# Xinran1205/LBM-Asynchronous

Measured on AMD Instinct MI355X. Metric: MLUPS, higher is better.
Workload: dtype f32

## Files before the change

lbm-asynchronous_amd/csrc/lbm_hip.hip:

```cpp
#include "../../include/lbm_hip.h"
#include "lbm_kernels.hip.h"

#include <hip/hip_runtime.h>
#include <hip/hip_ext.h>
#include <rccl/rccl.h>

#include <dlfcn.h>
#include <algorithm>

#include <atomic>
#include <condition_variable>
#include <cstdarg>
#include <cstdio>
#include <cstdlib>
#include <cstring>
#include <functional>
#include <mutex>
#include <thread>
#include <vector>

namespace {

constexpr int kMaxSlabs = 8;
constexpr int kPartSlots = lbm::kPartSlotsMax;
// ... 91 lines not shown
  LBM_RCCL_SYM(Recv, "ncclRecv");                    LBM_RCCL_SYM(AllReduce, "ncclAllReduce");
  LBM_RCCL_SYM(GetErrorString, "ncclGetErrorString");
#undef LBM_RCCL_SYM
  if (!ok) { r.handle = nullptr; return; }
  Dl_info di;
  if (dladdr(reinterpret_cast<void*>(r.GetVersion), &di) && di.dli_fname) {
    char real[512];
    const char* shown = realpath(di.dli_fname, real) ? real : di.dli_fname;
    strncpy(r.path, shown, sizeof(r.path) - 1);
  }
}

RcclApi* rccl() {
  std::call_once(g_rccl_once, rccl_bind);
  return g_rccl.handle ? &g_rccl : nullptr;
}

#define RCCL_OR_FAIL(ret)                                                       \
  RcclApi* rc_api_ = rccl();                                                    \
  if (!rc_api_) LBM_FAIL(ret, "RCCL is not available: %s", g_rccl_error)

constexpr int kMaxBandGroups = 3;

struct Slab {
  int device = 0;
  int row_first = 0;
  int rows = 0;
  int accel_row = lbm::kNoRow;
  int accel_row2 = lbm::kNoRow;
  float* lat_alloc[2] = {nullptr, nullptr};
  float* lat[2] = {nullptr, nullptr};
  unsigned char* mask_alloc = nullptr;
  unsigned char* mask = nullptr;
  float* partials = nullptr;
  double* tot_u = nullptr;
  double* scratch = nullptr;
  double* reduce_buf = nullptr;
  int* flushed_dev = nullptr;
  uint4* res_gran = nullptr;
  float* res_part = nullptr;
  int* res_status = nullptr;
  int* res_status_host = nullptr;
  float* frames = nullptr;
  lbm::probe_vec* probe_ring = nullptr;
  lbm::ProbeEntry* probe_table = nullptr;
  int probe_count = 0;
  hipGraphExec_t chunk_graph[2] = {nullptr, nullptr};
  hipStream_t compute = nullptr, comm = nullptr;
  hipEvent_t ev_boundary = nullptr, ev_halo = nullptr, ev_t0 = nullptr, ev_t1 = nullptr;
  hipEvent_t ev_interior[2] = {nullptr, nullptr};
  hipEvent_t ev_flush = nullptr;
  hipEvent_t ev_step = nullptr;
  hipEvent_t ev_fork = nullptr;
  hipEvent_t ev_x[2] = {nullptr, nullptr};
  hipStream_t group_extra[kMaxBandGroups - 1] = {nullptr, nullptr};
  hipEvent_t ev_gi[2][kMaxBandGroups] = {};
  hipEvent_t ev_gs[2] = {nullptr, nullptr};
  float* fresh_stage = nullptr;
  unsigned* fresh_arrived = nullptr;
  unsigned* fresh_id_src = nullptr;
  int* fresh_decision = nullptr;
  unsigned char* fresh_log = nullptr;
  hipEvent_t ev_fresh[2] = {nullptr, nullptr};
  ncclComm_t nccl = nullptr;
  lbm::SlotCounts slot_counts;
  int blocks_main = 0;
// ... 122 lines not shown
  Slab slab[kMaxSlabs];
  int cur = 0;
  int steps_done = 0;
  int capacity = 0;
  int fluid_cells = 0;
  int math_mode = LBM_MATH_EXACT;
  int halo = HALO_SELF;
  int halo_mode = LBM_HALO_SYNC;
  int rank = 0, world = 1;
  bool ranked = false;
  bool hosted = false;
  lbm_host_comm host_comm = {nullptr, nullptr, nullptr};
  float* host_send[2] = {nullptr, nullptr};
  float* host_recv[2] = {nullptr, nullptr};
  int row_first = 0, row_count = 0;
  int slot_fill = 0;
  long part_stride = 0;
  bool vec4 = false;
  int neigh = 0;
  int nts = 1;
  int snake = 0;
  int fuse2 = 0;
  int pass_steps = 2;
  int prefetch = 0;
  int xcd_chunk = 0;
  int use_stepk = 0;
  int packed = 0;
  int halo_lanes = 1;
  int lds_windows = 0;
  int band_rows = 8, n_strips = 0;
  int band_groups = 1;
  bool groups_forked = false;
  int lane_cells = 4;
  SlabTeam* team = nullptr;
  int use_graph = 0;
  GraphBuilder* builder = nullptr;
  int resident = 0;
  int resident_min_steps = 16;
  int resident_bands = 0;
  int resident_joint = 0;
  int resident_rows = 4;
  int resident_group = 1;
  int resident_one_xcd = 0;
  long long resident_timeout = 0;
  bool resident_used = false;
  int tile_steps = 0;
  int tile_shape = 0;
  lbm_batch* batch = nullptr;
  int frame_every = 0;
  int frame_slots = 0;
  int frame_ord0 = 0;
  long long frames_written = 0;
  long long frames_read = 0;
  std::vector<lbm_probe> probe_cells;
  int probe_every = 0;
  int probe_slots = 0;
  int probe_ord0 = 0;
  long long probes_written = 0;
  long long probes_read = 0;
  lbm::SteadyState* steady_state = nullptr;
  int* steady_stop_host = nullptr;
  hipEvent_t ev_steady[2] = {nullptr, nullptr};
};

struct lbm_batch {
  std::vector<lbm_ctx*> members;
// ... 156 lines not shown
  return q_kernel(c, stream, reinterpret_cast<const void*>(kernel), dim3(waves), dim3(64), args, done);
}

int launch_stepk(lbm_ctx* c, int s, hipStream_t stream, int k, int row_first, int row_end, int band_rows,
                 int band_pitch, int band_count, int part_offset, bool accel_after, hipEvent_t done = nullptr) {
  Slab& sl = c->slab[s];
  if (band_count <= 0) return LBM_SUCCESS;
  lbm::StepKArgs a;
  a.src = sl.lat[c->cur];
  a.dst = sl.lat[c->cur ^ 1];
  a.mask = sl.mask;
  a.plane_stride = c->plane_stride;
  a.row_pitch = c->row_pitch;
  a.pitch = c->pitch;
  a.nx = c->p.nx;
  a.rows = sl.rows;
  a.wrap = (c->halo == HALO_SELF) ? 1 : 0;
  a.band_rows = band_rows;
  a.row_first = row_first;
  a.band_pitch = band_pitch;
  a.row_end = row_end;
  a.n_strips = c->n_strips;
  a.n_bands = band_count;
  a.chunk = c->xcd_chunk;
  a.halo_lanes = c->halo_lanes;
  a.accel_row = sl.accel_row;
  a.accel_row2 = sl.accel_row2;
  a.accel_after = accel_after ? 1 : 0;
  a.omega = c->p.omega;
  a.a1 = c->p.density * c->p.accel / 9.f;
  a.a2 = c->p.density * c->p.accel / 36.f;
  a.partials = sl.partials + (long)c->slot_fill * c->part_stride + part_offset;
  a.slot_stride = c->part_stride;
  int waves = c->n_strips * band_count;
  if (a.chunk > 0) {
    const int chunks = band_count * ceil_div(c->n_strips, a.chunk);
    waves = 8 * ceil_div(chunks, 8) * a.chunk;
  }
  typedef void (*fn)(const lbm::StepKArgs);
#define LBM_K_ROW(M, N) {{lbm::stepk_stream<M, N, 4, 2, false>, lbm::stepk_stream<M, N, 4, 2, true>}, \
                         {lbm::stepk_stream<M, N, 4, 3, false>, lbm::stepk_stream<M, N, 4, 3, true>}, \
                         {lbm::stepk_stream<M, N, 4, 4, false>, lbm::stepk_stream<M, N, 4, 4, false>}}
  static const fn table[2][2][3][2] = {{LBM_K_ROW(0, false), LBM_K_ROW(0, true)}, {LBM_K_ROW(1, false), LBM_K_ROW(1, true)}};
#undef LBM_K_ROW
#define LBM_PK(N, KK, PF) {lbm::stepk_pk<N, KK, (PF && KK < 4), 0>, lbm::stepk_pk<N, KK, (PF && KK < 4), 1>, lbm::stepk_pk<N, KK, PF, (KK > 2 ? 2 : 1)>}
#define LBM_PK_ROW(N) {{LBM_PK(N, 2, false), LBM_PK(N, 2, true)}, {LBM_PK(N, 3, false), LBM_PK(N, 3, true)}, \
                       {LBM_PK(N, 4, false), LBM_PK(N, 4, true)}}
  static const fn table_pk[2][3][2][3] = {LBM_PK_ROW(false), LBM_PK_ROW(true)};
#undef LBM_PK_ROW
#undef LBM_PK
#define LBM_PK1(N, KK, PF) {lbm::stepk_pk<N, KK, (PF && KK < 4), 0, false, 1>, lbm::stepk_pk<N, KK, PF, 1, false, 1>}
#define LBM_PK1_ROW(N) {{LBM_PK1(N, 2, false), LBM_PK1(N, 2, true)}, {LBM_PK1(N, 3, false), LBM_PK1(N, 3, true)}, \
                        {LBM_PK1(N, 4, false), LBM_PK1(N, 4, true)}}
  static const fn table_pk1[2][3][2][2] = {LBM_PK1_ROW(false), LBM_PK1_ROW(true)};
#undef LBM_PK1_ROW
#undef LBM_PK1
  const int lds_windows = c->lds_windows < k ? c->lds_windows : k - 1;
  const bool packed = c->packed != 0;
  const fn kernel = (packed && c->lane_cells == 2) ? table_pk1[c->nts][k - 2][c->prefetch ? 1 : 0][lds_windows ? 1 : 0]
                    : packed ? table_pk[c->nts][k - 2][c->prefetch ? 1 : 0][lds_windows]
                           : table[c->math_mode == LBM_MATH_EXACT ? 0 : 1][c->nts][k - 2][c->prefetch ? 1 : 0];
  void* args[] = {&a};
  return q_kernel(c, stream, reinterpret_cast<const void*>(kernel), dim3(waves), dim3(64), args, done);
}

int launch_pass(lbm_ctx* c, int s, hipStream_t stream, int k, int row_first, int row_end, int band_rows,
                int band_pitch, int band_count, int part_offset, bool accel_after, hipEvent_t done = nullptr) {
  if ((c->lane_cells == 4 && (k > 2 || c->prefetch || c->xcd_chunk || c->use_stepk || c->packed)) ||
      (c->lane_cells == 2 && c->packed))
    return launch_stepk(c, s, stream, k, row_first, row_end, band_rows, band_pitch, band_count, part_offset, accel_after, done);
  return launch_step2(c, s, stream, row_first, row_end, band_rows, band_pitch, band_count, part_offset, accel_after, done);
}

int tile_count_for(const lbm_params* p, int shape) {
  return ceil_div(p->nx, kTileShapes[shape].tw) * ceil_div(p->ny, kTileShapes[shape].th);
}
int tile_count(const lbm_ctx* c) {
  const TileShape& t = kTileShapes[c->tile_shape];
  return ceil_div(c->p.nx, t.tw) * ceil_div(c->slab[0].rows, t.th);
}

int launch_tile(lbm_ctx* c, hipStream_t stream, int n_steps, bool accel_after) {
  Slab& sl = c->slab[0];
  lbm::TileArgs a;
  a.src = sl.lat[c->cur];
  a.dst = sl.lat[c->cur ^ 1];
  a.mask = sl.mask;
  a.plane_stride = c->plane_stride;
  a.row_pitch = c->row_pitch;
  a.pitch = c->pitch;
  a.nx = c->p.nx;
  a.ny = sl.rows;
  a.n_steps = n_steps;
// ... 966 lines not shown
          return LBM_SUCCESS;
        }) != LBM_SUCCESS)
      return LBM_FAILURE;
    for (int s = 0; s < c->n_slabs; s++)
      c->slab[s].slot_counts.n[c->slot_fill] = freshest ? c->slab[s].blocks_main + c->slab[s].blocks_boundary : blocks_for_rows(c, c->slab[s].rows);
    c->cur ^= 1;
    c->slot_fill += 1;
    if (!last && freshest && !force_never && fresh_exchange(c, c->cur, (m + 1) & 1, (unsigned)(c->steps_done + m + 1) + 1u) != LBM_SUCCESS)
      return LBM_FAILURE;
    if (!last && exchange_halos(c, depth, c->cur, c->cur ^ 1, slot) != LBM_SUCCESS) return LBM_FAILURE;
    if (c->slot_fill >= kPartSlots - 1 || last) {
      if (flush_partials(c, flushed_upto) != LBM_SUCCESS) return LBM_FAILURE;
      flushed_upto += c->slot_fill;
      c->slot_fill = 0;
    }
  }
  c->steps_done += n_steps;

  for (int s = 0; s < c->n_slabs; s++) {
    Slab& sl = c->slab[s];
    HIP_TRY(LBM_FAILURE, hipSetDevice(sl.device));
    for (int i = 0; i < 2; i++) HIP_TRY(LBM_FAILURE, hipStreamWaitEvent(sl.compute, sl.ev_x[i], 0));
  }
  return kernel_ms ? read_step_timing(c, n_steps, kernel_ms) : LBM_SUCCESS;
}

void free_slab(Slab& sl) {
  if (hipSetDevice(sl.device) != hipSuccess) return;
  for (int i = 0; i < 2; i++)
    if (sl.chunk_graph[i]) { (void)hipGraphExecDestroy(sl.chunk_graph[i]); sl.chunk_graph[i] = nullptr; }
  if (sl.nccl && g_rccl.CommDestroy) g_rccl.CommDestroy(sl.nccl);
  for (int i = 0; i < 2; i++) if (sl.lat_alloc[i]) (void)hipFree(sl.lat_alloc[i]);
  if (sl.mask_alloc) (void)hipFree(sl.mask_alloc);
  if (sl.partials) (void)hipFree(sl.partials);
  if (sl.tot_u) (void)hipFree(sl.tot_u);
  if (sl.scratch) (void)hipFree(sl.scratch);
  if (sl.reduce_buf) (void)hipFree(sl.reduce_buf);
  if (sl.flushed_dev) (void)hipFree(sl.flushed_dev);
  if (sl.fresh_stage) (void)hipFree(sl.fresh_stage);
  if (sl.fresh_arrived) (void)hipFree(sl.fresh_arrived);
  if (sl.fresh_id_src) (void)hipFree(sl.fresh_id_src);
  if (sl.fresh_decision) (void)hipFree(sl.fresh_decision);
  if (sl.fresh_log) (void)hipFree(sl.fresh_log);
  for (int i = 0; i < 2; i++) if (sl.ev_fresh[i]) (void)hipEventDestroy(sl.ev_fresh[i]);
  if (sl.res_gran) (void)hipFree(sl.res_gran);
  if (sl.res_part) (void)hipFree(sl.res_part);
  if (sl.res_status) (void)hipFree(sl.res_status);
  if (sl.res_status_host) (void)hipHostFree(sl.res_status_host);
  if (sl.frames) (void)hipFree(sl.frames);
  if (sl.probe_ring) (void)hipFree(sl.probe_ring);
  if (sl.probe_table) (void)hipFree(sl.probe_table);
  if (sl.ev_boundary) (void)hipEventDestroy(sl.ev_boundary);
  if (sl.ev_halo) (void)hipEventDestroy(sl.ev_halo);
  for (int i = 0; i < 2; i++) if (sl.ev_interior[i]) (void)hipEventDestroy(sl.ev_interior[i]);
  if (sl.ev_flush) (void)hipEventDestroy(sl.ev_flush);
  if (sl.ev_step) (void)hipEventDestroy(sl.ev_step);
  if (sl.ev_fork) (void)hipEventDestroy(sl.ev_fork);
  for (int i = 0; i < 2; i++) if (sl.ev_x[i]) (void)hipEventDestroy(sl.ev_x[i]);
  if (sl.ev_t0) (void)hipEventDestroy(sl.ev_t0);
  if (sl.ev_t1) (void)hipEventDestroy(sl.ev_t1);
  for (int i = 0; i < 2; i++) {
    if (sl.ev_gs[i]) (void)hipEventDestroy(sl.ev_gs[i]);
    for (int g = 0; g < kMaxBandGroups; g++) if (sl.ev_gi[i][g]) (void)hipEventDestroy(sl.ev_gi[i][g]);
  }
  for (int g = 0; g < kMaxBandGroups - 1; g++) if (sl.group_extra[g]) (void)hipStreamDestroy(sl.group_extra[g]);
  if (sl.compute) (void)hipStreamDestroy(sl.compute);
// ... 73 lines not shown
      HIP_TRY(LBM_FAILURE, hipMalloc(&tile_buf.p, tn));
      unsigned char* tile_dev = tile_buf.as<unsigned char>();
      HIP_TRY(LBM_FAILURE, hipMemcpyAsync(tile_dev, t8.data(), tn, hipMemcpyHostToDevice, sl.compute));
      hipLaunchKernelGGL(lbm::mask_from_tile, dim3(ceil_div((long)p.nx * mrows, 256)), dim3(256), 0, sl.compute, tile_dev,
                         obst.tile_nx, obst.tile_ny, sl.mask_alloc, p.nx, c->pitch, sl.row_first - kMaskHalo, mrows, p.ny);
      HIP_TRY(LBM_FAILURE, hipGetLastError());
      HIP_TRY(LBM_FAILURE, hipStreamSynchronize(sl.compute));
    } else {
      long chunk_rows = (32L << 20) / ((long)p.nx * sizeof(int));
      if (chunk_rows < 1) chunk_rows = 1;
      DeviceTemp stage_buf;
      HIP_TRY(LBM_FAILURE, hipMalloc(&stage_buf.p, (size_t)chunk_rows * p.nx * sizeof(int)));
      int* stage = stage_buf.as<int>();
      for (int r = 0; r < mrows;) {
        long src_row;
        int run = mrows - r;
        if (obst.kind == OBST_ROWS) {
          src_row = (long)(sl.row_first - c->row_first) + r;
        } else {
          const int g = ((sl.row_first - kMaskHalo + r) % p.ny + p.ny) % p.ny;
          src_row = g;
          if (run > p.ny - g) run = p.ny - g;
        }
        if (run > chunk_rows) run = (int)chunk_rows;
        HIP_TRY(LBM_FAILURE, hipMemcpyAsync(stage, obst.data + (size_t)src_row * p.nx, (size_t)run * p.nx * sizeof(int),
                                            hipMemcpyHostToDevice, sl.compute));
        hipLaunchKernelGGL(lbm::mask_from_int, dim3(ceil_div((long)p.nx * run, 256)), dim3(256), 0, sl.compute, stage,
                           sl.mask_alloc + (size_t)r * c->pitch, p.nx, c->pitch, run);
        HIP_TRY(LBM_FAILURE, hipGetLastError());
        HIP_TRY(LBM_FAILURE, hipStreamSynchronize(sl.compute));
        r += run;
      }
    }
    unsigned long long* cnt = reinterpret_cast<unsigned long long*>(sl.scratch);
    HIP_TRY(LBM_FAILURE, hipMemsetAsync(cnt, 0, sizeof(unsigned long long), sl.compute));
    hipLaunchKernelGGL(lbm::count_blocked, dim3(ceil_div((long)c->pitch * sl.rows, 256 * 16)), dim3(256), 0, sl.compute,
                       sl.mask, (long)c->pitch * sl.rows, cnt);
    HIP_TRY(LBM_FAILURE, hipGetLastError());
    unsigned long long blocked = 0;
    HIP_TRY(LBM_FAILURE, hipMemcpyAsync(&blocked, cnt, sizeof(blocked), hipMemcpyDeviceToHost, sl.compute));
    HIP_TRY(LBM_FAILURE, hipStreamSynchronize(sl.compute));
    sl.fluid_cells = (long)p.nx * sl.rows - (long)blocked;
  }

  if (!cells_aos) {
    const float r0 = p.density * 4.f / 9.f;
    const float r1 = p.density / 9.f;
    const float r2 = p.density / 36.f;
    hipLaunchKernelGGL(lbm::init_equilibrium, dim3(ceil_div((long)p.nx * sl.rows, 256)), dim3(256), 0,
                       sl.compute, sl.lat[0], c->plane_stride, c->row_pitch, p.nx, sl.rows, r0, r1, r2);
    HIP_TRY(LBM_FAILURE, hipGetLastError());
  } else {
    const int chunk_rows = (int)(((64L << 20) / ((long)p.nx * lbm::kQ * sizeof(float))) > 0
                                     ? ((64L << 20) / ((long)p.nx * lbm::kQ * sizeof(float)))
                                     : 1);
    DeviceTemp stage_buf;
    HIP_TRY(LBM_FAILURE, hipMalloc(&stage_buf.p, (size_t)chunk_rows * p.nx * lbm::kQ * sizeof(float)));
    float* stage = stage_buf.as<float>();
    for (int r0 = 0; r0 < sl.rows; r0 += chunk_rows) {
      const int nr = (sl.rows - r0 < chunk_rows) ? sl.rows - r0 : chunk_rows;
      const size_t n = (size_t)nr * p.nx * lbm::kQ;
      HIP_TRY(LBM_FAILURE, hipMemcpyAsync(stage, cells_aos + (size_t)(sl.row_first - (obst.local_cells ? c->row_first : 0) + r0) * p.nx * lbm::kQ,
                                          n * sizeof(float), hipMemcpyHostToDevice, sl.compute));
      hipLaunchKernelGGL(lbm::aos_to_soa, dim3(ceil_div((long)n, 256)), dim3(256), 0, sl.compute, stage,
                         sl.lat[0], c->plane_stride, c->row_pitch, p.nx, r0, nr);
      HIP_TRY(LBM_FAILURE, hipGetLastError());
// ... 116 lines not shown
      const bool in_halo = (c->halo != HALO_SELF) && ((local < 0 && local >= -kMaskHalo) || (local >= sl.rows && local < sl.rows + kMaskHalo));
      if (owned || in_halo) {
        if (sl.accel_row == lbm::kNoRow || owned) { if (sl.accel_row != lbm::kNoRow) sl.accel_row2 = sl.accel_row; sl.accel_row = local; }
        else sl.accel_row2 = local;
      }
    }
    if (c->halo == HALO_SELF) {
      sl.blocks_main = blocks_for_rows(c, sl.rows);
      sl.blocks_boundary = 0;
    } else {
      if (sl.rows < 2) {
        raise_error(__LINE__, "lbm_create: a slab needs at least 2 rows");
        delete c;
        return nullptr;
      }
      sl.blocks_main = blocks_for_rows(c, sl.rows - 2);
      sl.blocks_boundary = blocks_for_rows(c, 2);
    }
    if (sl.blocks_main + sl.blocks_boundary > max_blocks) max_blocks = sl.blocks_main + sl.blocks_boundary;
  }
  c->fuse2 = plan.fuse2;
  c->lane_cells = plan.lane_cells;
  c->pass_steps = plan.pass_steps;
  c->halo_lanes = ceil_div(c->pass_steps, c->lane_cells);
  c->n_strips = ceil_div(params->nx / c->lane_cells > 0 ? params->nx / c->lane_cells : 1, 64 - 2 * c->halo_lanes);
  c->packed = env_int("LBM_PACKED", 1) ? 1 : 0;
  c->lds_windows = env_int("LBM_LDS_WINDOWS", (c->packed && c->pass_steps == 4) ? 2 : 0);
  if (c->lds_windows < 0 || c->lds_windows > 2 || !c->packed) c->lds_windows = 0;
  c->prefetch = env_int("LBM_PREFETCH", (c->lane_cells == 4 && (c->pass_steps == 3 || (c->pass_steps == 4 && c->lds_windows == 2))) ? 1 : 0) ? 1 : 0;
  const bool many_rounds = (long)c->n_strips * ceil_div(c->row_count / n_slabs, 24) >= 16L * 1024;
  c->xcd_chunk = env_int("LBM_XCD_CHUNK", (c->pass_steps >= 3 && many_rounds) ? c->n_strips : 0);
  if (c->xcd_chunk < 0 || c->xcd_chunk > c->n_strips) c->xcd_chunk = 0;
  c->use_stepk = env_int("LBM_STEPK", 0) ? 1 : 0;

  if (!halo_on && n_slabs == 1 && c->fuse2 && !c->use_graph) {
    c->band_groups = env_int("LBM_BAND_GROUPS", (c->lane_cells == 4 && c->pass_steps == 4) ? 2 : 1);
    if (c->band_groups < 1) c->band_groups = 1;
    if (c->band_groups > kMaxBandGroups) c->band_groups = kMaxBandGroups;
  }
  {
    int pick = (params->nx <= 7168) ? 5 : (params->nx <= 8192 ? 7 : (params->nx <= 12288 ? 5 : 4));
    const long resident = 256L * 4 * 5;
    const long slab_rows = (n_slabs > 1 || world > 1) ? (c->row_count / n_slabs) - 4 : c->row_count;
    const long rows_eff = slab_rows > 1 ? slab_rows : 1;
    if (c->lane_cells == 2 && (long)c->n_strips * ceil_div(rows_eff, 8) < 5 * resident) {
      const long lo = 3;
      long best_cost = -1;
      for (int k = 1; k <= 4; k++) {
        long b = (rows_eff * c->n_strips + k * resident - 1) / (k * resident);
        if (b < lo) b = lo;
        if (b > 32) b = 32;
        const long rounds = ((long)c->n_strips * ceil_div(rows_eff, b) + resident - 1) / resident;
        const long cost = rounds * (b + 2);
        if (best_cost < 0 || cost < best_cost) { best_cost = cost; pick = (int)b; }
      }
    }
    if (c->lane_cells == 2 && c->pass_steps >= 3) {
      const long interior = (n_slabs > 1 || world > 1 || halo_on) ? rows_eff + 4 - 2 * c->pass_steps : rows_eff;
      long b = ((interior > 1 ? interior : 1) * c->n_strips + 2047) / 2048;
      pick = (int)(b < 3 ? 3 : (b > 64 ? 64 : b));
    }
    if (c->lane_cells == 4 && c->pass_steps >= 3) {
      const int groups = c->band_groups;
      const long interior = (n_slabs > 1 || world > 1 || halo_on) ? rows_eff + 4 - 2 * c->pass_steps
                                                                  : (groups > 1 ? rows_eff / groups - 2 * c->pass_steps : rows_eff);
      const long r_int = interior > 1 ? interior : 1;
// ... 1210 lines not shown
```

lbm-asynchronous_amd/csrc/lbm_kernels.hip.h:

```cpp
#pragma once
#include <hip/hip_runtime.h>

#include <type_traits>

namespace lbm {

constexpr int kBlock = 256;
constexpr int kQ = 9;
constexpr int kNoRow = -1000000;

constexpr float kCsq = 1.f / 3.f;
constexpr float kTwoCsq = 2.f * kCsq;
constexpr float kTwoCsqSq = 2.f * kCsq * kCsq;
constexpr float kW0 = 4.f / 9.f;
constexpr float kW1 = 1.f / 9.f;
constexpr float kW2 = 1.f / 36.f;

struct StepArgs {
  const float* src;
  float* dst;
  const unsigned char* mask;
  long plane_stride;
  int pitch;
  long row_pitch;
// ... 343 lines not shown
  int band_pitch;
  int row_end;
  int n_strips;
  int accel_row;
  int accel_after;
  float omega, a1, a2;
  float* partials1;
  float* partials2;
};

constexpr int kStripQuads = 62;

template <int MATH, int SPEED = 0>
__device__ __forceinline__ void relax_cell(const float (&t)[kQ], bool blocked, bool lid, float omega, float a1,
                                           float a2, float (&r)[kQ], float& speed, bool want_speed = true) {
  speed = 0.f;
  if (blocked) {
    bounce(t, r);
  } else {
    if constexpr (MATH == 0) collide_exact<SPEED>(t, omega, r, speed, want_speed);
    else collide<false>(t, omega, r, speed, want_speed);
    if (lid) accelerate(r, a1, a2);
  }
}

template <int C>
struct RowPull {
  typedef float vec __attribute__((ext_vector_type(C)));
  vec v[kQ];
  unsigned m;
};

template <int C>
__device__ __forceinline__ RowPull<C> pull_row(const Step2Args& a, int r, int x0) {
  typedef typename RowPull<C>::vec vec;
  const long ps = a.plane_stride;
  const int rs = (r == 0 && a.wrap) ? a.rows - 1 : r - 1;
  const int rn = (r == a.rows - 1 && a.wrap) ? 0 : r + 1;
  const float* c_row = a.src + (long)r * a.row_pitch + x0;
  const float* sb = a.src + (long)rs * a.row_pitch + x0;
  const float* nb = a.src + (long)rn * a.row_pitch + x0;
  RowPull<C> p;
  p.v[0] = *reinterpret_cast<const vec*>(c_row);
  p.v[1] = *reinterpret_cast<const vec*>(c_row + 1 * ps);
  p.v[3] = *reinterpret_cast<const vec*>(c_row + 3 * ps);
  p.v[2] = *reinterpret_cast<const vec*>(sb + 2 * ps);
  p.v[5] = *reinterpret_cast<const vec*>(sb + 5 * ps);
  p.v[6] = *reinterpret_cast<const vec*>(sb + 6 * ps);
  p.v[4] = *reinterpret_cast<const vec*>(nb + 4 * ps);
  p.v[7] = *reinterpret_cast<const vec*>(nb + 7 * ps);
  p.v[8] = *reinterpret_cast<const vec*>(nb + 8 * ps);
  const unsigned char* mp = a.mask + (long)r * a.pitch + x0;
  if constexpr (C == 4) p.m = *reinterpret_cast<const unsigned*>(mp);
  else if constexpr (C == 2) p.m = *reinterpret_cast<const unsigned short*>(mp);
  else p.m = *mp;
  return p;
}

__device__ __forceinline__ int wrap_row(int r, int rows, int wrap) {
  if (wrap) {
    if (r < 0) r += rows;
    if (r >= rows) r -= rows;
  }
  return r;
}

template <int MATH, bool NTS, int C>
__global__ __launch_bounds__(64) void step2_stream(const Step2Args a) {
  typedef typename RowPull<C>::vec vec;
  const int lane = threadIdx.x;
  const int strip = blockIdx.x % a.n_strips;
  const int units_x = a.nx / C;
  const int y0 = a.row_first + (int)(blockIdx.x / a.n_strips) * a.band_pitch;
  const int band_n = min(a.band_rows, a.row_end - y0);

  const int ux_raw = strip * kStripQuads + lane - 1;
  int ux = ux_raw % units_x;
  if (ux < 0) ux += units_x;
  const int x0 = ux * C;
  const bool out_lane = (lane >= 1) && (lane <= kStripQuads) && (ux_raw < units_x);
  const long ps = a.plane_stride;

  float w256[3][C];
  float w013[3][C];
  float n256[3][C];
  unsigned m_prev = 0;
  float sum1 = 0.f, sum2 = 0.f;

// ... 83 lines not shown

  sum1 = wave_sum(sum1);
  sum2 = wave_sum(sum2);
  if (lane == 0) {
    a.partials1[blockIdx.x] = sum1;
    a.partials2[blockIdx.x] = sum2;
  }
}

struct StepKArgs {
  const float* src;
  float* dst;
  const unsigned char* mask;
  long plane_stride;
  long row_pitch;
  int pitch;
  int nx;
  int rows;
  int wrap;
  int band_rows;
  int row_first;
  int band_pitch;
  int row_end;
  int n_strips;
  int n_bands;
  int chunk;
  int halo_lanes;
  int accel_row;
  int accel_row2;
  int accel_after;
  float omega, a1, a2;
  float* partials;
  long slot_stride;
};

template <int C>
struct Window {
  float w256[3][C];
  float w013[3][C];
  float n256[3][C];
  unsigned m;
};

template <int MATH, bool NTS, int C, int K, bool PREFETCH>
__global__ __launch_bounds__(64, (K >= 3 || PREFETCH || MATH == 0) ? 2 : 3) void stepk_stream(const StepKArgs a) {
  static_assert(K >= 2 && K <= 4 && (C == 4 || K == 2), "one halo lane per side covers K <= C steps");
  typedef typename RowPull<C>::vec vec;
  const int lane = threadIdx.x;
  int strip, band;
  if (a.chunk > 0) {
    const int xcd = blockIdx.x & 7, j = blockIdx.x >> 3;
    const int chunks_per_band = (a.n_strips + a.chunk - 1) / a.chunk;
    const int g = (j / a.chunk) * 8 + xcd;
    band = g / chunks_per_band;
    strip = (g - band * chunks_per_band) * a.chunk + j % a.chunk;
    if (band >= a.n_bands || strip >= a.n_strips) return;
  } else {
    strip = blockIdx.x % a.n_strips;
    band = blockIdx.x / a.n_strips;
  }
  const int wave_id = band * a.n_strips + strip;
  const int units_x = a.nx / C;
  const int y0 = a.row_first + band * a.band_pitch;
  const int band_n = min(a.band_rows, a.row_end - y0);

  const int H = a.halo_lanes;
// ... 210 lines not shown
#pragma unroll
  for (int i = 0; i < 3; i++) {
    const float a = (i == 0) ? a1 : a2;
    const f2 up = f2{r[plus[i]].x + a, r[plus[i]].y + a}, dn = f2{r[minus[i]].x - a, r[minus[i]].y - a};
    r[plus[i]] = f2{g0 ? up.x : r[plus[i]].x, g1 ? up.y : r[plus[i]].y};
    r[minus[i]] = f2{g0 ? dn.x : r[minus[i]].x, g1 ? dn.y : r[minus[i]].y};
  }
}
__device__ __forceinline__ void relax_pair_guard_path(const f2 (&f)[kQ], bool b0, bool b1, float omega, f2 (&r)[kQ],
                                                      bool want_speed, float& sp0, float& sp1) {
#pragma unroll
  for (int c = 0; c < 2; c++) {
    if (!(c == 0 ? b0 : b1)) {
      float ts[kQ], rs[kQ], speed;
#pragma unroll
      for (int k = 0; k < kQ; k++) ts[k] = f[k][c];
      relax_cell<0, 1>(ts, false, false, omega, 0.f, 0.f, rs, speed, want_speed);
#pragma unroll
      for (int k = 0; k < kQ; k++) r[k][c] = rs[k];
      if (c == 0) sp0 = speed; else sp1 = speed;
    }
  }
}
__device__ __forceinline__ void relax_pair_fixup(const f2 (&f)[kQ], bool ok, unsigned blocked, bool lid, float omega,
                                                 float a1, float a2, f2 (&r)[kQ], bool want_speed, float& sp0, float& sp1) {
  if (!ok || lid || blocked != 0) {
    const bool b0 = (blocked & 0xffu) != 0, b1 = (blocked & 0xff00u) != 0;
    if (!ok) relax_pair_guard_path(f, b0, b1, omega, r, want_speed, sp0, sp1);
    if (lid) accelerate_select(r, !b0, !b1, a1, a2);
    if (blocked != 0) bounce_select(f, b0, b1, r, sp0, sp1);
  }
}

__device__ __forceinline__ float relax_pair_exact(const f2 (&f)[kQ], unsigned blocked, bool lid, float omega,
                                                  float a1, float a2, f2 (&r)[kQ], bool want_speed) {
  f2 u_sq;
  const bool ok = relax_pair_core(f, omega, r, u_sq);
  float sp0 = 0.f, sp1 = 0.f;
  if (want_speed) {
    sp0 = __builtin_amdgcn_sqrtf(u_sq.x);
    sp1 = __builtin_amdgcn_sqrtf(u_sq.y);
  }
  relax_pair_fixup(f, ok, blocked, lid, omega, a1, a2, r, want_speed, sp0, sp1);
  return sp0 + sp1;
}

__device__ __forceinline__ float relax_quad_exact(const f2 (&f0)[kQ], const f2 (&f1)[kQ], unsigned blocked, bool lid,
                                                  float omega, float a1, float a2, f2 (&r0)[kQ], f2 (&r1)[kQ],
                                                  bool want_speed) {
  f2 usq0, usq1;
  const bool ok0 = relax_pair_core(f0, omega, r0, usq0);
  const bool ok1 = relax_pair_core(f1, omega, r1, usq1);
  float sp[4] = {0.f, 0.f, 0.f, 0.f};
  if (want_speed) {
    sp[0] = __builtin_amdgcn_sqrtf(usq0.x);  sp[1] = __builtin_amdgcn_sqrtf(usq0.y);
    sp[2] = __builtin_amdgcn_sqrtf(usq1.x);  sp[3] = __builtin_amdgcn_sqrtf(usq1.y);
  }
  relax_pair_fixup(f0, ok0, blocked & 0xffffu, lid, omega, a1, a2, r0, want_speed, sp[0], sp[1]);
  relax_pair_fixup(f1, ok1, blocked >> 16, lid, omega, a1, a2, r1, want_speed, sp[2], sp[3]);
  return (sp[0] + sp[1]) + (sp[2] + sp[3]);
}

template <int NP, int P>
__device__ __forceinline__ f2 pair_from_west(const f2 (&a)[NP], float W) {
  if constexpr (P == 0) return f2{W, a[0].x};
  else return f2{a[P - 1].y, a[P].x};
}
template <int NP, int P>
__device__ __forceinline__ f2 pair_from_east(const f2 (&a)[NP], float E) {
  if constexpr (P == NP - 1) return f2{a[P].y, E};
  else return f2{a[P].y, a[P + 1].x};
}

template <int NP>
struct WindowPk {
  f2 w256[3][NP];
  f2 w013[3][NP];
  f2 n256[3][NP];
  unsigned m;
};

template <bool NTS, int K, bool PREFETCH, int LW, bool QUAD = false, int NP = 2>
__global__ __launch_bounds__(64, NP == 1 ? (K > 2 ? 3 : (PREFETCH ? 2 : 4)) : 2) void stepk_pk(const StepKArgs a) {
  static_assert(K >= 2 && K <= 4 && LW >= 0 && LW <= K - 1 && (NP == 2 || !QUAD), "halo_lanes * C >= K is the host's job");
  constexpr int C = 2 * NP;
  typedef typename RowPull<C>::vec vec;
  __shared__ vec lds_win[LW > 0 ? LW : 1][9][64];
  const int lane = threadIdx.x;
  int strip, band;
  if (a.chunk > 0) {
    const int xcd = blockIdx.x & 7, j = blockIdx.x >> 3;
    const int chunks_per_band = (a.n_strips + a.chunk - 1) / a.chunk;
    const int g = (j / a.chunk) * 8 + xcd;
    band = g / chunks_per_band;
    strip = (g - band * chunks_per_band) * a.chunk + j % a.chunk;
    if (band >= a.n_bands || strip >= a.n_strips) return;
  } else {
    strip = blockIdx.x % a.n_strips;
    band = blockIdx.x / a.n_strips;
  }
  const int wave_id = band * a.n_strips + strip;
  const int units_x = a.nx / C;
  const int y0 = a.row_first + band * a.band_pitch;
  const int band_n = min(a.band_rows, a.row_end - y0);

  const int H = a.halo_lanes;
  const int ux_raw = strip * (64 - 2 * H) + lane - H;
  int ux = ux_raw % units_x;
  if (ux < 0) ux += units_x;
  const int x0 = ux * C;
  const bool out_lane = (lane >= H) && (lane < 64 - H) && (ux_raw < units_x);
  const long ps = a.plane_stride;

  Step2Args pa;
  pa.src = a.src;  pa.mask = a.mask;  pa.plane_stride = a.plane_stride;  pa.row_pitch = a.row_pitch;
// ... 3 lines not shown
#pragma unroll
  for (int s = 0; s < K - 1; s++) {
    win[s].m = 0;
#pragma unroll
    for (int q = 0; q < 3; q++)
#pragma unroll
      for (int p = 0; p < NP; p++) win[s].w256[q][p] = win[s].w013[q][p] = win[s].n256[q][p] = splat2(0.f);
  }
  if constexpr (LW > 0) {
#pragma unroll
    for (int l = 0; l < LW; l++)
#pragma unroll
      for (int q = 0; q < 9; q++) {
        vec z;
#pragma unroll
        for (int j = 0; j < C; j++) z[j] = 0.f;
        lds_win[l][q][lane] = z;
      }
  }
  float sum[K];
#pragma unroll
  for (int s = 0; s < K; s++) sum[s] = 0.f;

  auto pairs_of = [](const vec& v, f2 (&o)[NP]) {
#pragma unroll
    for (int p = 0; p < NP; p++) o[p] = f2{v[2 * p], v[2 * p + 1]};
  };
  auto vec_of = [](const f2 (&c)[NP][kQ], int k) {
    vec o;
#pragma unroll
    for (int p = 0; p < NP; p++) { o[2 * p] = c[p][k].x;  o[2 * p + 1] = c[p][k].y; }
    return o;
  };
  auto relax_row = [&](const f2 (&in)[kQ][NP], unsigned m, bool lid, f2 (&out)[NP][kQ], bool own_row) {
    f2 t0[kQ];
#pragma unroll
    for (int k = 0; k < kQ; k++) t0[k] = in[k][0];
    if constexpr (NP == 1) {
      return relax_pair_exact(t0, m & 0xffffu, lid, a.omega, a.a1, a.a2, out[0], own_row);
    } else {
      f2 t1[kQ];
#pragma unroll
      for (int k = 0; k < kQ; k++) t1[k] = in[k][NP - 1];
      if constexpr (QUAD) {
        return relax_quad_exact(t0, t1, m, lid, a.omega, a.a1, a.a2, out[0], out[NP - 1], own_row);
      } else {
        const float s0 = relax_pair_exact(t0, m & 0xffffu, lid, a.omega, a.a1, a.a2, out[0], own_row);
        return s0 + relax_pair_exact(t1, m >> 16, lid, a.omega, a.a1, a.a2, out[NP - 1], own_row);
      }
    }
  };
  auto shifted = [](const f2 (&pl)[kQ][NP], const float (&W)[kQ], const float (&E)[kQ], f2 (&in)[kQ][NP]) {
#pragma unroll
    for (int k = 0; k < kQ; k++) {
      const bool west = (k == 1 || k == 5 || k == 8), east = (k == 3 || k == 6 || k == 7);
      if (west) {
        in[k][0] = pair_from_west<NP, 0>(pl[k], W[k]);
        if constexpr (NP == 2) in[k][NP - 1] = pair_from_west<NP, NP - 1>(pl[k], W[k]);
      } else if (east) {
        in[k][0] = pair_from_east<NP, 0>(pl[k], E[k]);
        if constexpr (NP == 2) in[k][NP - 1] = pair_from_east<NP, NP - 1>(pl[k], E[k]);
      } else {
#pragma unroll
        for (int p = 0; p < NP; p++) in[k][p] = pl[k][p];
      }
    }
  };

  const int n_iter = band_n + 2 * (K - 1);
  int r_next = wrap_row(y0 - (K - 1), a.rows, a.wrap);
  int r_hist[K];
#pragma unroll
  for (int s = 0; s < K; s++) r_hist[s] = 0;
  unsigned lid_hist = 0, own_hist = 0;
  RowPull<C> nextp;
  if constexpr (PREFETCH) nextp = pull_row<C>(pa, r_next, x0);

  auto row_iteration = [&](auto warm_c, const int i) {
    constexpr bool WARM = decltype(warm_c)::value;
    const int r = r_next;
    r_next = r + 1;
    if (a.wrap && r_next >= a.rows) r_next -= a.rows;
#pragma unroll
    for (int s = K - 1; s > 0; s--) r_hist[s] = r_hist[s - 1];
    r_hist[0] = r;
    lid_hist = (lid_hist << 1) | ((r == a.accel_row || r == a.accel_row2) ? 1u : 0u);
    own_hist = (own_hist << 1) | ((i >= K - 1 && i < band_n + K - 1) ? 1u : 0u);
    RowPull<C> p;
    if constexpr (PREFETCH) {
      p = nextp;
      if (i + 1 < n_iter) nextp = pull_row<C>(pa, r_next, x0);
    } else {
      p = pull_row<C>(pa, r, x0);
    }
    f2 cur[NP][kQ];
    {
      float W[kQ] = {}, E[kQ] = {};
      W[1] = lane_from_west<2>(p.v[1][C - 1]);  W[5] = lane_from_west<2>(p.v[5][C - 1]);  W[8] = lane_from_west<2>(p.v[8][C - 1]);
      E[3] = lane_from_east<2>(p.v[3][0]);      E[6] = lane_from_east<2>(p.v[6][0]);      E[7] = lane_from_east<2>(p.v[7][0]);
      f2 pl[kQ][NP], in[kQ][NP];
#pragma unroll
      for (int k = 0; k < kQ; k++) pairs_of(p.v[k], pl[k]);
      shifted(pl, W, E, in);
      const bool lid = (lid_hist & 1u) != 0;
      const bool own_row = (own_hist & 1u) != 0;
      const float sp = relax_row(in, p.m, lid, cur, own_row);
      if (own_row && out_lane) sum[0] += sp;
    }
    unsigned m_cur = p.m;

    bool alive = true;
    auto stage = [&](auto sc) {
      constexpr int s = decltype(sc)::value;
      constexpr bool in_lds = (s - 1) >= (K - 1 - LW);
      constexpr int li = in_lds ? (s - 1) - (K - 1 - LW) : 0;
      if (!alive) return;
      WindowPk<NP>& w = win[s - 1];
      const int ring = (i & 1) * 3;
      f2 nxt[NP][kQ];
      const bool active = WARM ? (i >= 2 * s) : true;
      if (active) {
        f2 pl[kQ][NP];
        constexpr int q256[3] = {2, 5, 6}, q013[3] = {0, 1, 3};
        if constexpr (in_lds) {
#pragma unroll
          for (int q = 0; q < 3; q++) {
            pairs_of(lds_win[li][ring + q][lane], pl[q256[q]]);
            pairs_of(lds_win[li][6 + q][lane], pl[q013[q]]);
          }
        } else {
#pragma unroll
          for (int q = 0; q < 3; q++)
#pragma unroll
            for (int p2 = 0; p2 < NP; p2++) { pl[q256[q]][p2] = w.w256[q][p2];  pl[q013[q]][p2] = w.w013[q][p2]; }
        }
#pragma unroll
        for (int p2 = 0; p2 < NP; p2++) { pl[4][p2] = cur[p2][4];  pl[7][p2] = cur[p2][7];  pl[8][p2] = cur[p2][8]; }
        float W[kQ] = {}, E[kQ] = {};
        W[1] = lane_from_west<2>(pl[1][NP - 1].y);  W[5] = lane_from_west<2>(pl[5][NP - 1].y);  W[8] = lane_from_west<2>(pl[8][NP - 1].y);
        E[3] = lane_from_east<2>(pl[3][0].x);       E[6] = lane_from_east<2>(pl[6][0].x);       E[7] = lane_from_east<2>(pl[7][0].x);
        f2 in[kQ][NP];
        shifted(pl, W, E, in);
        const bool last = (s == K - 1);
        const bool lid = ((lid_hist >> s) & 1u) != 0 && (!last || a.accel_after);
        const bool own_row = ((own_hist >> s) & 1u) != 0;
        const float sp = relax_row(in, w.m, lid, nxt, own_row);
        if (own_row && out_lane) sum[s] += sp;
      }
      const unsigned m_below = w.m;
      if constexpr (in_lds) {
        lds_win[li][ring + 0][lane] = vec_of(cur, 2);
        lds_win[li][ring + 1][lane] = vec_of(cur, 5);
        lds_win[li][ring + 2][lane] = vec_of(cur, 6);
        lds_win[li][6][lane] = vec_of(cur, 0);
        lds_win[li][7][lane] = vec_of(cur, 1);
        lds_win[li][8][lane] = vec_of(cur, 3);
      } else {
#pragma unroll
        for (int p2 = 0; p2 < NP; p2++) {
          w.w256[0][p2] = w.n256[0][p2];  w.w256[1][p2] = w.n256[1][p2];  w.w256[2][p2] = w.n256[2][p2];
          w.n256[0][p2] = cur[p2][2];     w.n256[1][p2] = cur[p2][5];     w.n256[2][p2] = cur[p2][6];
          w.w013[0][p2] = cur[p2][0];     w.w013[1][p2] = cur[p2][1];     w.w013[2][p2] = cur[p2][3];
        }
      }
      w.m = m_cur;
      if (!active) { alive = false; return; }
      m_cur = m_below;
#pragma unroll
      for (int p2 = 0; p2 < NP; p2++)
#pragma unroll
        for (int k = 0; k < kQ; k++) cur[p2][k] = nxt[p2][k];
      if (s == K - 1 && out_lane) {
        const int ro = r_hist[K - 1];
        float* d_row = a.dst + (long)ro * a.row_pitch + x0;
#pragma unroll
        for (int k = 0; k < kQ; k++) {
          const vec o = vec_of(cur, k);
          if constexpr (NTS) __builtin_nontemporal_store(o, reinterpret_cast<vec*>(d_row + k * ps));
          else *reinterpret_cast<vec*>(d_row + k * ps) = o;
// ... 814 lines not shown
  const float* p = partials + (long)blockIdx.x * slot_stride;
  const int n_part = counts.n[blockIdx.x];
  double acc = 0.0;
  for (int i = threadIdx.x; i < n_part; i += kBlock) acc += (double)p[i];
  sh[threadIdx.x] = acc;
  __syncthreads();
  for (int s = kBlock / 2; s > 0; s >>= 1) {
    if (threadIdx.x < s) sh[threadIdx.x] += sh[threadIdx.x + s];
    __syncthreads();
  }
  if (threadIdx.x == 0) tot_u[step_base + blockIdx.x] = sh[0];
}

__global__ void set_counter(int* p, int value) { *p = value; }
__global__ void advance_counter(int* p, int by) { *p += by; }

__global__ void mask_from_int(const int* src, unsigned char* dst, int nx, int pitch, int nrows) {
  const long i = (long)blockIdx.x * blockDim.x + threadIdx.x;
  if (i >= (long)nx * nrows) return;
  const int r = (int)(i / nx), x = (int)(i - (long)r * nx);
  dst[(long)r * pitch + x] = src[i] ? 1 : 0;
}

__global__ void mask_from_tile(const unsigned char* tile, int tnx, int tny, unsigned char* dst, int nx, int pitch,
                               int row0, int nrows, int ny) {
  const long i = (long)blockIdx.x * blockDim.x + threadIdx.x;
  if (i >= (long)nx * nrows) return;
  const int r = (int)(i / nx), x = (int)(i - (long)r * nx);
  int g = (row0 + r) % ny;
  if (g < 0) g += ny;
  dst[(long)r * pitch + x] = tile[(long)(g % tny) * tnx + (x % tnx)];
}

__global__ __launch_bounds__(256) void count_blocked(const unsigned char* mask, long n, unsigned long long* out) {
  __shared__ unsigned int sh[256];
  unsigned int acc = 0;
  const long base = ((long)blockIdx.x * 256 + threadIdx.x) * 16;
  for (int k = 0; k < 16; k++)
    if (base + k < n) acc += mask[base + k] ? 1u : 0u;
  sh[threadIdx.x] = acc;
  __syncthreads();
  for (int s = 128; s > 0; s >>= 1) {
    if (threadIdx.x < s) sh[threadIdx.x] += sh[threadIdx.x + s];
    __syncthreads();
  }
  if (threadIdx.x == 0 && sh[0]) atomicAdd(out, (unsigned long long)sh[0]);
}

__global__ void init_equilibrium(float* lat, long ps, long row_pitch, int nx, int rows, float r0,
                                 float r1, float r2) {
  const long j = (long)blockIdx.x * blockDim.x + threadIdx.x;
  if (j >= (long)nx * rows) return;
  const long row = j / nx;
  const long i = row * row_pitch + (j - row * nx);
  lat[i] = r0;
  lat[1 * ps + i] = r1;  lat[2 * ps + i] = r1;  lat[3 * ps + i] = r1;  lat[4 * ps + i] = r1;
  lat[5 * ps + i] = r2;  lat[6 * ps + i] = r2;  lat[7 * ps + i] = r2;  lat[8 * ps + i] = r2;
}

__global__ void aos_to_soa(const float* aos, float* lat, long ps, long row_pitch, int nx, int row0,
                           int nrows) {
  const long i = (long)blockIdx.x * blockDim.x + threadIdx.x;
  const long n = (long)nx * nrows * kQ;
  if (i >= n) return;
  const long cell = i / kQ;
  const int k = (int)(i - cell * kQ);
// ... 105 lines not shown
```

Measured before the change: 266,900.

## Precompute per-strip row obstacle classes to skip mask loads and bounce-back fixups

```diff
diff --git a/lbm-asynchronous_amd/csrc/lbm_hip.hip b/lbm-asynchronous_amd/csrc/lbm_hip.hip
--- a/lbm-asynchronous_amd/csrc/lbm_hip.hip
+++ b/lbm-asynchronous_amd/csrc/lbm_hip.hip
@@ -147,6 +147,8 @@
   float* lat[2] = {nullptr, nullptr};
   unsigned char* mask_alloc = nullptr;
   unsigned char* mask = nullptr;
+  unsigned char* row_class = nullptr;
+  int class_pitch = 0;
   float* partials = nullptr;
   double* tot_u = nullptr;
   double* scratch = nullptr;
@@ -335,6 +337,7 @@
   int band_groups = 1;
   bool groups_forked = false;
   int lane_cells = 4;
+  int obstacle_classes = 1;
   SlabTeam* team = nullptr;
   int use_graph = 0;
   GraphBuilder* builder = nullptr;
@@ -557,6 +560,10 @@
   a.a2 = c->p.density * c->p.accel / 36.f;
   a.partials = sl.partials + (long)c->slot_fill * c->part_stride + part_offset;
   a.slot_stride = c->part_stride;
+  const bool classes = c->obstacle_classes && c->packed && c->lane_cells == 4 && sl.row_class;
+  a.row_class = classes ? sl.row_class : nullptr;
+  a.class_pitch = sl.class_pitch;
+  a.class_halo = kMaskHalo;
   int waves = c->n_strips * band_count;
   if (a.chunk > 0) {
     const int chunks = band_count * ceil_div(c->n_strips, a.chunk);
@@ -568,10 +575,12 @@
                          {lbm::stepk_stream<M, N, 4, 4, false>, lbm::stepk_stream<M, N, 4, 4, false>}}
   static const fn table[2][2][3][2] = {{LBM_K_ROW(0, false), LBM_K_ROW(0, true)}, {LBM_K_ROW(1, false), LBM_K_ROW(1, true)}};
 #undef LBM_K_ROW
-#define LBM_PK(N, KK, PF) {lbm::stepk_pk<N, KK, (PF && KK < 4), 0>, lbm::stepk_pk<N, KK, (PF && KK < 4), 1>, lbm::stepk_pk<N, KK, PF, (KK > 2 ? 2 : 1)>}
-#define LBM_PK_ROW(N) {{LBM_PK(N, 2, false), LBM_PK(N, 2, true)}, {LBM_PK(N, 3, false), LBM_PK(N, 3, true)}, \
-                       {LBM_PK(N, 4, false), LBM_PK(N, 4, true)}}
-  static const fn table_pk[2][3][2][3] = {LBM_PK_ROW(false), LBM_PK_ROW(true)};
+#define LBM_PK(N, KK, PF, CL) {lbm::stepk_pk<N, KK, (PF && KK < 4), 0, false, 2, CL>, lbm::stepk_pk<N, KK, (PF && KK < 4), 1, false, 2, CL>, \
+                              lbm::stepk_pk<N, KK, PF, (KK > 2 ? 2 : 1), false, 2, CL>}
+#define LBM_PK_ROW(N, CL) {{LBM_PK(N, 2, false, CL), LBM_PK(N, 2, true, CL)}, {LBM_PK(N, 3, false, CL), LBM_PK(N, 3, true, CL)}, \
+                           {LBM_PK(N, 4, false, CL), LBM_PK(N, 4, true, CL)}}
+  static const fn table_pk[2][2][3][2][3] = {{LBM_PK_ROW(false, false), LBM_PK_ROW(true, false)},
+                                             {LBM_PK_ROW(false, true), LBM_PK_ROW(true, true)}};
 #undef LBM_PK_ROW
 #undef LBM_PK
 #define LBM_PK1(N, KK, PF) {lbm::stepk_pk<N, KK, (PF && KK < 4), 0, false, 1>, lbm::stepk_pk<N, KK, PF, 1, false, 1>}
@@ -583,7 +592,7 @@
   const int lds_windows = c->lds_windows < k ? c->lds_windows : k - 1;
   const bool packed = c->packed != 0;
   const fn kernel = (packed && c->lane_cells == 2) ? table_pk1[c->nts][k - 2][c->prefetch ? 1 : 0][lds_windows ? 1 : 0]
-                    : packed ? table_pk[c->nts][k - 2][c->prefetch ? 1 : 0][lds_windows]
+                    : packed ? table_pk[classes ? 1 : 0][c->nts][k - 2][c->prefetch ? 1 : 0][lds_windows]
                            : table[c->math_mode == LBM_MATH_EXACT ? 0 : 1][c->nts][k - 2][c->prefetch ? 1 : 0];
   void* args[] = {&a};
   return q_kernel(c, stream, reinterpret_cast<const void*>(kernel), dim3(waves), dim3(64), args, done);
@@ -1616,6 +1625,7 @@
   if (sl.nccl && g_rccl.CommDestroy) g_rccl.CommDestroy(sl.nccl);
   for (int i = 0; i < 2; i++) if (sl.lat_alloc[i]) (void)hipFree(sl.lat_alloc[i]);
   if (sl.mask_alloc) (void)hipFree(sl.mask_alloc);
+  if (sl.row_class) (void)hipFree(sl.row_class);
   if (sl.partials) (void)hipFree(sl.partials);
   if (sl.tot_u) (void)hipFree(sl.tot_u);
   if (sl.scratch) (void)hipFree(sl.scratch);
@@ -1755,6 +1765,15 @@
         r += run;
       }
     }
+    if (c->n_strips > 0 && p.nx % c->lane_cells == 0) {
+      sl.class_pitch = (mrows + 4 + 3) / 4 * 4;
+      const size_t class_bytes = (size_t)c->n_strips * sl.class_pitch;
+      HIP_TRY(LBM_FAILURE, hipMalloc(&sl.row_class, class_bytes));
+      HIP_TRY(LBM_FAILURE, hipMemsetAsync(sl.row_class, 0, class_bytes, sl.compute));
+      hipLaunchKernelGGL(lbm::strip_row_classes, dim3(mrows, c->n_strips), dim3(64), 0, sl.compute, sl.mask_alloc, c->pitch,
+                         p.nx, c->lane_cells, c->halo_lanes, sl.row_class, sl.class_pitch);
+      HIP_TRY(LBM_FAILURE, hipGetLastError());
+    }
     unsigned long long* cnt = reinterpret_cast<unsigned long long*>(sl.scratch);
     HIP_TRY(LBM_FAILURE, hipMemsetAsync(cnt, 0, sizeof(unsigned long long), sl.compute));
     hipLaunchKernelGGL(lbm::count_blocked, dim3(ceil_div((long)c->pitch * sl.rows, 256 * 16)), dim3(256), 0, sl.compute,
@@ -1937,6 +1956,7 @@
   c->xcd_chunk = env_int("LBM_XCD_CHUNK", (c->pass_steps >= 3 && many_rounds) ? c->n_strips : 0);
   if (c->xcd_chunk < 0 || c->xcd_chunk > c->n_strips) c->xcd_chunk = 0;
   c->use_stepk = env_int("LBM_STEPK", 0) ? 1 : 0;
+  c->obstacle_classes = env_int("LBM_OBSTACLE_CLASSES", 1) ? 1 : 0;
 
   if (!halo_on && n_slabs == 1 && c->fuse2 && !c->use_graph) {
     c->band_groups = env_int("LBM_BAND_GROUPS", (c->lane_cells == 4 && c->pass_steps == 4) ? 2 : 1);
diff --git a/lbm-asynchronous_amd/csrc/lbm_kernels.hip.h b/lbm-asynchronous_amd/csrc/lbm_kernels.hip.h
--- a/lbm-asynchronous_amd/csrc/lbm_kernels.hip.h
+++ b/lbm-asynchronous_amd/csrc/lbm_kernels.hip.h
@@ -399,7 +399,7 @@
 };
 
 template <int C>
-__device__ __forceinline__ RowPull<C> pull_row(const Step2Args& a, int r, int x0) {
+__device__ __forceinline__ RowPull<C> pull_row(const Step2Args& a, int r, int x0, bool want_mask = true) {
   typedef typename RowPull<C>::vec vec;
   const long ps = a.plane_stride;
   const int rs = (r == 0 && a.wrap) ? a.rows - 1 : r - 1;
@@ -417,10 +417,13 @@
   p.v[4] = *reinterpret_cast<const vec*>(nb + 4 * ps);
   p.v[7] = *reinterpret_cast<const vec*>(nb + 7 * ps);
   p.v[8] = *reinterpret_cast<const vec*>(nb + 8 * ps);
-  const unsigned char* mp = a.mask + (long)r * a.pitch + x0;
-  if constexpr (C == 4) p.m = *reinterpret_cast<const unsigned*>(mp);
-  else if constexpr (C == 2) p.m = *reinterpret_cast<const unsigned short*>(mp);
-  else p.m = *mp;
+  p.m = 0;
+  if (want_mask) {
+    const unsigned char* mp = a.mask + (long)r * a.pitch + x0;
+    if constexpr (C == 4) p.m = *reinterpret_cast<const unsigned*>(mp);
+    else if constexpr (C == 2) p.m = *reinterpret_cast<const unsigned short*>(mp);
+    else p.m = *mp;
+  }
   return p;
 }
 
@@ -570,6 +573,9 @@
   float omega, a1, a2;
   float* partials;
   long slot_stride;
+  const unsigned char* row_class;
+  int class_pitch;
+  int class_halo;
 };
 
 template <int C>
@@ -846,8 +852,28 @@
   }
 }
 
+__device__ __forceinline__ void relax_pair_fixup_cls(const f2 (&f)[kQ], bool ok, unsigned blocked, unsigned cls, bool lid,
+                                                     float omega, float a1, float a2, f2 (&r)[kQ], bool want_speed,
+                                                     float& sp0, float& sp1) {
+  constexpr int opp[kQ] = {0, 3, 4, 1, 2, 7, 8, 5, 6};
+  const bool b0 = (blocked & 0xffu) != 0, b1 = (blocked & 0xff00u) != 0;
+  if (!ok) relax_pair_guard_path(f, b0, b1, omega, r, want_speed, sp0, sp1);
+  if (lid) accelerate_select(r, !b0, !b1, a1, a2);
+  if (cls & 1u) {
+#pragma unroll
+    for (int k = 0; k < kQ; k++) r[k].x = b0 ? f[opp[k]].x : r[k].x;
+    sp0 = b0 ? 0.f : sp0;
+  }
+  if (cls & 2u) {
+#pragma unroll
+    for (int k = 0; k < kQ; k++) r[k].y = b1 ? f[opp[k]].y : r[k].y;
+    sp1 = b1 ? 0.f : sp1;
+  }
+}
+
+template <bool CLS = false>
 __device__ __forceinline__ float relax_pair_exact(const f2 (&f)[kQ], unsigned blocked, bool lid, float omega,
-                                                  float a1, float a2, f2 (&r)[kQ], bool want_speed) {
+                                                  float a1, float a2, f2 (&r)[kQ], bool want_speed, unsigned cls = 0) {
   f2 u_sq;
   const bool ok = relax_pair_core(f, omega, r, u_sq);
   float sp0 = 0.f, sp1 = 0.f;
@@ -855,13 +881,15 @@
     sp0 = __builtin_amdgcn_sqrtf(u_sq.x);
     sp1 = __builtin_amdgcn_sqrtf(u_sq.y);
   }
-  relax_pair_fixup(f, ok, blocked, lid, omega, a1, a2, r, want_speed, sp0, sp1);
+  if constexpr (CLS) relax_pair_fixup_cls(f, ok, blocked, cls, lid, omega, a1, a2, r, want_speed, sp0, sp1);
+  else relax_pair_fixup(f, ok, blocked, lid, omega, a1, a2, r, want_speed, sp0, sp1);
   return sp0 + sp1;
 }
 
+template <bool CLS = false>
 __device__ __forceinline__ float relax_quad_exact(const f2 (&f0)[kQ], const f2 (&f1)[kQ], unsigned blocked, bool lid,
                                                   float omega, float a1, float a2, f2 (&r0)[kQ], f2 (&r1)[kQ],
-                                                  bool want_speed) {
+                                                  bool want_speed, unsigned cls = 0) {
   f2 usq0, usq1;
   const bool ok0 = relax_pair_core(f0, omega, r0, usq0);
   const bool ok1 = relax_pair_core(f1, omega, r1, usq1);
@@ -870,8 +898,13 @@
     sp[0] = __builtin_amdgcn_sqrtf(usq0.x);  sp[1] = __builtin_amdgcn_sqrtf(usq0.y);
     sp[2] = __builtin_amdgcn_sqrtf(usq1.x);  sp[3] = __builtin_amdgcn_sqrtf(usq1.y);
   }
-  relax_pair_fixup(f0, ok0, blocked & 0xffffu, lid, omega, a1, a2, r0, want_speed, sp[0], sp[1]);
-  relax_pair_fixup(f1, ok1, blocked >> 16, lid, omega, a1, a2, r1, want_speed, sp[2], sp[3]);
+  if constexpr (CLS) {
+    relax_pair_fixup_cls(f0, ok0, blocked & 0xffffu, cls & 3u, lid, omega, a1, a2, r0, want_speed, sp[0], sp[1]);
+    relax_pair_fixup_cls(f1, ok1, blocked >> 16, cls >> 2, lid, omega, a1, a2, r1, want_speed, sp[2], sp[3]);
+  } else {
+    relax_pair_fixup(f0, ok0, blocked & 0xffffu, lid, omega, a1, a2, r0, want_speed, sp[0], sp[1]);
+    relax_pair_fixup(f1, ok1, blocked >> 16, lid, omega, a1, a2, r1, want_speed, sp[2], sp[3]);
+  }
   return (sp[0] + sp[1]) + (sp[2] + sp[3]);
 }
 
@@ -894,7 +927,7 @@
   unsigned m;
 };
 
-template <bool NTS, int K, bool PREFETCH, int LW, bool QUAD = false, int NP = 2>
+template <bool NTS, int K, bool PREFETCH, int LW, bool QUAD = false, int NP = 2, bool CLS = false>
 __global__ __launch_bounds__(64, NP == 1 ? (K > 2 ? 3 : (PREFETCH ? 2 : 4)) : 2) void stepk_pk(const StepKArgs a) {
   static_assert(K >= 2 && K <= 4 && LW >= 0 && LW <= K - 1 && (NP == 2 || !QUAD), "halo_lanes * C >= K is the host's job");
   constexpr int C = 2 * NP;
@@ -964,21 +997,21 @@
     for (int p = 0; p < NP; p++) { o[2 * p] = c[p][k].x;  o[2 * p + 1] = c[p][k].y; }
     return o;
   };
-  auto relax_row = [&](const f2 (&in)[kQ][NP], unsigned m, bool lid, f2 (&out)[NP][kQ], bool own_row) {
+  auto relax_row = [&](const f2 (&in)[kQ][NP], unsigned m, unsigned cls, bool lid, f2 (&out)[NP][kQ], bool own_row) {
     f2 t0[kQ];
 #pragma unroll
     for (int k = 0; k < kQ; k++) t0[k] = in[k][0];
     if constexpr (NP == 1) {
-      return relax_pair_exact(t0, m & 0xffffu, lid, a.omega, a.a1, a.a2, out[0], own_row);
+      return relax_pair_exact<CLS>(t0, m & 0xffffu, lid, a.omega, a.a1, a.a2, out[0], own_row, cls & 3u);
     } else {
       f2 t1[kQ];
 #pragma unroll
       for (int k = 0; k < kQ; k++) t1[k] = in[k][NP - 1];
       if constexpr (QUAD) {
-        return relax_quad_exact(t0, t1, m, lid, a.omega, a.a1, a.a2, out[0], out[NP - 1], own_row);
+        return relax_quad_exact<CLS>(t0, t1, m, lid, a.omega, a.a1, a.a2, out[0], out[NP - 1], own_row, cls);
       } else {
-        const float s0 = relax_pair_exact(t0, m & 0xffffu, lid, a.omega, a.a1, a.a2, out[0], own_row);
-        return s0 + relax_pair_exact(t1, m >> 16, lid, a.omega, a.a1, a.a2, out[NP - 1], own_row);
+        const float s0 = relax_pair_exact<CLS>(t0, m & 0xffffu, lid, a.omega, a.a1, a.a2, out[0], own_row, cls & 3u);
+        return s0 + relax_pair_exact<CLS>(t1, m >> 16, lid, a.omega, a.a1, a.a2, out[NP - 1], own_row, cls >> 2);
       }
     }
   };
@@ -1005,8 +1038,25 @@
 #pragma unroll
   for (int s = 0; s < K; s++) r_hist[s] = 0;
   unsigned lid_hist = 0, own_hist = 0;
+  typedef const unsigned __attribute__((address_space(4))) class_word;
+  class_word* const cls_words =
+      reinterpret_cast<class_word*>(reinterpret_cast<uintptr_t>(a.row_class)) + (CLS ? (long)strip * (a.class_pitch >> 2) : 0);
+  auto class_of = [&](int row) -> unsigned {
+    const int idx = min(max(row + a.class_halo, 0), a.class_pitch - 1);
+    return (cls_words[idx >> 2] >> ((idx & 3) * 8)) & 0xfu;
+  };
+  auto row_after = [&](int row) {
+    row++;
+    if (a.wrap && row >= a.rows) row -= a.rows;
+    return row;
+  };
+  unsigned cls_hist = 0, cls_next = 0, cls_pulled = 0;
+  if constexpr (CLS) cls_next = class_of(r_next);
   RowPull<C> nextp;
-  if constexpr (PREFETCH) nextp = pull_row<C>(pa, r_next, x0);
+  if constexpr (PREFETCH) {
+    nextp = pull_row<C>(pa, r_next, x0, !CLS || cls_next != 0);
+    if constexpr (CLS) { cls_pulled = cls_next;  cls_next = class_of(row_after(r_next)); }
+  }
 
   auto row_iteration = [&](auto warm_c, const int i) {
     constexpr bool WARM = decltype(warm_c)::value;
@@ -1021,9 +1071,14 @@
     RowPull<C> p;
     if constexpr (PREFETCH) {
       p = nextp;
-      if (i + 1 < n_iter) nextp = pull_row<C>(pa, r_next, x0);
+      if constexpr (CLS) cls_hist = (cls_hist << 4) | cls_pulled;
+      if (i + 1 < n_iter) {
+        nextp = pull_row<C>(pa, r_next, x0, !CLS || cls_next != 0);
+        if constexpr (CLS) { cls_pulled = cls_next;  cls_next = class_of(row_after(r_next)); }
+      }
     } else {
-      p = pull_row<C>(pa, r, x0);
+      p = pull_row<C>(pa, r, x0, !CLS || cls_next != 0);
+      if constexpr (CLS) { cls_hist = (cls_hist << 4) | cls_next;  cls_next = class_of(r_next); }
     }
     f2 cur[NP][kQ];
     {
@@ -1036,7 +1091,7 @@
       shifted(pl, W, E, in);
       const bool lid = (lid_hist & 1u) != 0;
       const bool own_row = (own_hist & 1u) != 0;
-      const float sp = relax_row(in, p.m, lid, cur, own_row);
+      const float sp = relax_row(in, p.m, cls_hist & 0xfu, lid, cur, own_row);
       if (own_row && out_lane) sum[0] += sp;
     }
     unsigned m_cur = p.m;
@@ -1076,7 +1131,7 @@
         const bool last = (s == K - 1);
         const bool lid = ((lid_hist >> s) & 1u) != 0 && (!last || a.accel_after);
         const bool own_row = ((own_hist >> s) & 1u) != 0;
-        const float sp = relax_row(in, w.m, lid, nxt, own_row);
+        const float sp = relax_row(in, w.m, (cls_hist >> (4 * s)) & 0xfu, lid, nxt, own_row);
         if (own_row && out_lane) sum[s] += sp;
       }
       const unsigned m_below = w.m;
@@ -1957,6 +2012,19 @@
   dst[(long)r * pitch + x] = tile[(long)(g % tny) * tnx + (x % tnx)];
 }
 
+__global__ __launch_bounds__(64) void strip_row_classes(const unsigned char* mask, int pitch, int nx, int cells,
+                                                        int halo_lanes, unsigned char* out, int class_pitch) {
+  const int row = blockIdx.x, strip = blockIdx.y, lane = threadIdx.x;
+  const int units_x = nx / cells;
+  int ux = (strip * (64 - 2 * halo_lanes) + lane - halo_lanes) % units_x;
+  if (ux < 0) ux += units_x;
+  const unsigned char* mp = mask + (long)row * pitch + ux * cells;
+  unsigned cls = 0;
+  for (int p = 0; p < cells; p++)
+    if (__ballot(mp[p] != 0) != 0) cls |= 1u << p;
+  if (lane == 0) out[(long)strip * class_pitch + row] = (unsigned char)cls;
+}
+
 __global__ __launch_bounds__(256) void count_blocked(const unsigned char* mask, long n, unsigned long long* out) {
   __shared__ unsigned int sh[256];
   unsigned int acc = 0;
```

Result: no change. 264,600 (-0.9%).
